# hassony2/homan

Measured on AMD Instinct MI355X. Metric: optimisation iters/sec (30-frame 256^2 clip), higher is better.
Workload: dtype f32

## Files before the change

### homan_amd/csrc/geometry.hip

```cpp
#include "hm_common.h"

__global__ __launch_bounds__(256) void k_rigid_fwd(const float* __restrict__ mesh, const float* __restrict__ rot6d,
                                                   const float* __restrict__ trans, const float* __restrict__ scale,
                                                   int abs_scale, int N, int V, float* __restrict__ rotmat,
                                                   float* __restrict__ verts, int clip_len)
{
    __shared__ float R[9];
    const int n = blockIdx.y;
    if (threadIdx.x == 0) {
        float r[9];
        rot6d_to_mat(rot6d + n * 6, r);
#pragma unroll
        for (int k = 0; k < 9; ++k) R[k] = r[k];
        if (blockIdx.x == 0 && rotmat)
#pragma unroll
            for (int k = 0; k < 9; ++k) rotmat[n * 9 + k] = r[k];
    }
    __syncthreads();
    const int v = blockIdx.x * blockDim.x + threadIdx.x;
    if (v >= V) return;
    float s = scale[n / clip_len];
    if (abs_scale) s = fabsf(s);
    const float* m = mesh + ((long)n * V + v) * 3;
    const float x = s * m[0], y = s * m[1], z = s * m[2];
// ... 140 lines not shown
        __syncthreads();
        if (threadIdx.x == 0) {
#pragma unroll
            for (int k = 0; k < 13; ++k) tot[k] = 0.f;
            for (unsigned c = 0; c < gridDim.y; ++c)
#pragma unroll
                for (int k = 0; k < 13; ++k) tot[k] += red13[c * 13 + k];
        }
    }
    }
    if (threadIdx.x == 0) {
        float dr6[6];
        rot6d_backward(rot6d + n * 6, tot, dr6);
#pragma unroll
        for (int k = 0; k < 6; ++k) g_rot6d[n * 6 + k] = dr6[k];
#pragma unroll
        for (int k = 0; k < 3; ++k) g_trans[n * 3 + k] = tot[9 + k];
        if (g_scale_part) g_scale_part[n] = (abs_scale && sraw < 0.f) ? -tot[12] : tot[12];
    }
    HM_STAMP_END(sil.parts ? 1 : 0);
}

struct SmoothIn { const float* verts; float w; };
template <int NV, int MAXT>
__global__ __launch_bounds__(MAXT) void k_rigid_bwd_x(const float* __restrict__ mesh, const float* __restrict__ rot6d,
                                                     const float* __restrict__ scale, int abs_scale, RigidTerms terms,
                                                     SilGather sil, SmoothIn sm, int N, int V, float* __restrict__ g_rot6d,
                                                     float* __restrict__ g_trans, float* __restrict__ g_scale_part,
                                                     float* __restrict__ partials, unsigned int* __restrict__ frame_cnt,
                                                     int clip_len, double magic)
{
    HM_LATENCY_KERNEL();
    HM_STAMP_START(1);
    __shared__ double red13d[16 * 13];
    __shared__ int s_flag;
    const int n = blockIdx.x;
    float R[9];
    rot6d_to_mat(rot6d + n * 6, R);
    const float sraw = scale[n / clip_len];
    const float s = abs_scale ? fabsf(sraw) : sraw;
    const int fl = n % clip_len;
    const long row = (long)V * 3;
    const long scnt = (long)(clip_len - 1) * row;
    const float inv_cnt = scnt > 0 ? 1.0f / (float)scnt : 0.f;
    int vv[NV];
    bool ok[NV];
    int a0[NV], a1[NV];
    float m[NV][3], cv[NV][3], tv[NV][5][3], nb[NV][2][3];
#pragma unroll
    for (int j = 0; j < NV; ++j) {
        vv[j] = ((int)blockIdx.y * NV + j) * (int)blockDim.x + (int)threadIdx.x;
        ok[j] = vv[j] < V;
        const int v = ok[j] ? vv[j] : 0;
        const long o = ((long)n * V + v) * 3;
        a0[j] = sil.parts ? sil.adj_off[v] : 0;
        a1[j] = sil.parts ? sil.adj_off[v + 1] : 0;
#pragma unroll
        for (int c = 0; c < 3; ++c) {
            m[j][c] = mesh[o + c];
            cv[j][c] = sil.parts ? sil.cam_verts[o + c] : 0.f;
        }
#pragma unroll
        for (int k = 0; k < 5; ++k)
#pragma unroll
            for (int c = 0; c < 3; ++c) tv[j][k][c] = terms.p[k] ? terms.p[k][o + c] : 0.f;
#pragma unroll
        for (int c = 0; c < 3; ++c) {
            nb[j][0][c] = (sm.verts && fl + 1 < clip_len) ? sm.verts[o + row + c] : 0.f;
            nb[j][1][c] = (sm.verts && fl >= 1) ? sm.verts[o - row + c] : 0.f;
        }
    }
    float sv[NV][3];
#pragma unroll
    for (int j = 0; j < NV; ++j)
#pragma unroll
        for (int c = 0; c < 3; ++c) sv[j][c] = sm.verts ? sm.verts[((long)n * V + (ok[j] ? vv[j] : 0)) * 3 + c] : 0.f;
    int item[NV][8];
#pragma unroll
    for (int j = 0; j < NV; ++j)
#pragma unroll
        for (int k = 0; k < 8; ++k) item[j][k] = (ok[j] && a0[j] + k < a1[j]) ? sil.adj_items[a0[j] + k] : -1;
    double su[NV], sw[NV];
    {
        const double2* pf = reinterpret_cast<const double2*>(sil.parts + (long)n * sil.F * 6);
        double2 g2[NV][8];
#pragma unroll
        for (int j = 0; j < NV; ++j)
#pragma unroll
            for (int k = 0; k < 8; ++k) g2[j][k] = item[j][k] >= 0 ? pf[item[j][k]] : make_double2(0.0, 0.0);
#pragma unroll
        for (int j = 0; j < NV; ++j) {
            su[j] = 0.0; sw[j] = 0.0;
#pragma unroll
            for (int k = 0; k < 8; ++k) { su[j] += g2[j][k].x; sw[j] += g2[j][k].y; }
            for (int a = a0[j] + 8; ok[j] && a < a1[j]; ++a) {
                const double2 g = pf[sil.adj_items[a]];
                su[j] += g.x; sw[j] += g.y;
            }
        }
    }
    double accd[13];
#pragma unroll
    for (int k = 0; k < 13; ++k) accd[k] = 0.0;
#pragma unroll
    for (int j = 0; j < NV; ++j) {
        if (!ok[j]) continue;
        float gf[3] = {0.f, 0.f, 0.f}, gt[3];
        if (sm.verts) {
#pragma unroll
            for (int c = 0; c < 3; ++c) {
                float g = 0.f;
                if (fl + 1 < clip_len) { const float d = nb[j][0][c] - sv[j][c]; g -= d; }
                if (fl >= 1) g += sv[j][c] - nb[j][1][c];
                gf[c] += sm.w * (2.0f * g * inv_cnt);
            }
        }
#pragma unroll
        for (int k = 0; k < 5; ++k)
            if (terms.p[k]) {
                gf[0] += terms.w[k] * tv[j][k][0]; gf[1] += terms.w[k] * tv[j][k][1]; gf[2] += terms.w[k] * tv[j][k][2];
            }
        if (sil.parts) {
            const float gu = (float)su[j], gv = (float)sw[j];
            const float* k = sil.K + n * 9;
            const float x = cv[j][0], y = cv[j][1], z = cv[j][2];
            const float zz = z + 1e-9f;
            const float du0 = gu * (2.0f / sil.orig_size), dv0 = -gv * (2.0f / sil.orig_size);
            const float dxn = k[0] * du0 + k[3] * dv0;
            const float dyn = k[1] * du0 + k[4] * dv0;
            gf[0] += dxn / zz;
            gf[1] += dyn / zz;
            gf[2] += -(dxn * x + dyn * y) / (zz * zz);
        }
        gt[0] = gf[0] + 0.f; gt[1] = gf[1] + 0.f; gt[2] = gf[2] + 0.f;
        const float dm[3] = {R[0] * gf[0] + R[1] * gf[1] + R[2] * gf[2], R[3] * gf[0] + R[4] * gf[1] + R[5] * gf[2],
                             R[6] * gf[0] + R[7] * gf[1] + R[8] * gf[2]};
#pragma unroll
        for (int i = 0; i < 3; ++i)
#pragma unroll
            for (int q = 0; q < 3; ++q) accd[3 * i + q] += hm_quant((s * m[j][i]) * gt[q], magic);
#pragma unroll
        for (int q = 0; q < 3; ++q) accd[9 + q] += hm_quant(gt[q], magic);
        accd[12] += hm_quant(m[j][0] * dm[0] + m[j][1] * dm[1] + m[j][2] * dm[2], magic);
    }
    hm_block_sum_n_f64<13>(accd, red13d);
    if (gridDim.y > 1) {
        double* rec = reinterpret_cast<double*>(partials + ((long)n * gridDim.y + blockIdx.y) * 32);
        if (threadIdx.x == 0) {
#pragma unroll
            for (int k = 0; k < 13; ++k) __hip_atomic_store(rec + k, accd[k], __ATOMIC_RELAXED, __HIP_MEMORY_SCOPE_AGENT);
        }
        if (!hm_last_block(frame_cnt + n, gridDim.y, &s_flag)) return;
        if (threadIdx.x < 13 * gridDim.y)
            red13d[threadIdx.x] = __hip_atomic_load(reinterpret_cast<const double*>(partials + ((long)n * gridDim.y + threadIdx.x / 13) * 32) + threadIdx.x % 13,
                                                    __ATOMIC_RELAXED, __HIP_MEMORY_SCOPE_AGENT);
        __syncthreads();
        if (threadIdx.x == 0) {
#pragma unroll
            for (int k = 0; k < 13; ++k) accd[k] = 0.0;
            for (unsigned c = 0; c < gridDim.y; ++c)
#pragma unroll
                for (int k = 0; k < 13; ++k) accd[k] += red13d[c * 13 + k];
        }
    }
    if (threadIdx.x == 0) {
        float tot[13], dr6[6];
#pragma unroll
        for (int k = 0; k < 13; ++k) tot[k] = (float)accd[k];
        rot6d_backward(rot6d + n * 6, tot, dr6);
#pragma unroll
        for (int k = 0; k < 6; ++k) g_rot6d[n * 6 + k] = dr6[k];
#pragma unroll
        for (int k = 0; k < 3; ++k) g_trans[n * 3 + k] = tot[9 + k];
        if (g_scale_part) g_scale_part[n] = (abs_scale && sraw < 0.f) ? -tot[12] : tot[12];
    }
    HM_STAMP_END(1);
}

__global__ void k_scale_by(const float* __restrict__ in, const float* __restrict__ s, long n, float* __restrict__ out)
{
    const long i = (long)blockIdx.x * blockDim.x + threadIdx.x;
    if (i < n) out[i] = s[0] * in[i];
}
__global__ void k_sum_small(const float* __restrict__ parts, int n, float w0, const float* __restrict__ extra, float w1,
                            float* __restrict__ out)
{
    __shared__ float red[16];
    const int c = blockIdx.x;
    float a = 0.f;
    for (int i = threadIdx.x; i < n; i += blockDim.x) a += parts[(long)c * n + i];
    a = hm_block_sum(a, red);
    if (threadIdx.x == 0) out[c] = w0 * a + (extra ? w1 * extra[c] : 0.f);
}

extern "C" {
int hm_sum_small_clips(const float* parts, int n, float w0, const float* extra, float w1, float* out, int nclips,
                       hipStream_t stream)
{
    HM_CHECK_ARG(parts && out && n > 0 && nclips > 0);
    hipLaunchKernelGGL(k_sum_small, dim3(nclips), dim3(64), 0, stream, parts, n, w0, extra, w1, out);
    return hm_launch_status();
}
int hm_rigid_fwd_clips(const float* mesh, const float* rot6d, const float* trans, const float* scale, int abs_scale, int N,
                       int V, float* rotmat, float* verts, int clip_len, hipStream_t stream)
{
    HM_CHECK_ARG(mesh && rot6d && trans && scale && verts && N > 0 && V > 0 && HM_CLIP_LEN_OK(N, clip_len));
    hipLaunchKernelGGL(k_rigid_fwd, dim3(hm_cdiv(V, 256), N), dim3(256), 0, stream, mesh, rot6d, trans, scale,
                       abs_scale, N, V, rotmat, verts, clip_len ? clip_len : N);
    return hm_launch_status();
}
int hm_rigid_fwd(const float* mesh, const float* rot6d, const float* trans, const float* scale, int abs_scale, int N,
                 int V, float* rotmat, float* verts, hipStream_t stream)
{
    return hm_rigid_fwd_clips(mesh, rot6d, trans, scale, abs_scale, N, V, rotmat, verts, 0, stream);
}
#define RIGID_MAX_CHUNKS 16
size_t hm_rigid_workspace_bytes(int N) { return (((size_t)N * 4 + 255) & ~(size_t)255) + (size_t)N * RIGID_MAX_CHUNKS * 32 * 4; }
static int rigid_bwd_launch(const float* mesh, const float* rot6d, const float* scale, int abs_scale,
                            const float* const* g_terms, const float* weights, int n_terms, SilGather sil,
                            const float* g_rigid, const float* g_frame, int frame_stride, float frame_scale, int N, int V,
                            float* g_mesh, float* g_rot6d, float* g_trans, float* g_scale_part, void* workspace,
                            int clip_len, int exact, int sum_log2q, SmoothIn smooth, hipStream_t stream)
{
    HM_CHECK_ARG(sum_log2q <= 0 && sum_log2q >= -60);
    HM_CHECK_ARG(mesh && rot6d && scale && g_rot6d && g_trans && N > 0 && V > 0 && HM_CLIP_LEN_OK(N, clip_len));
    HM_CHECK_ARG(n_terms >= 0 && n_terms <= 5 && (n_terms == 0 || (g_terms && weights)));
    HM_CHECK_ARG(!g_frame || frame_stride >= 3);
    HM_CHECK_ARG(HM_ALIGNED(workspace, 8));
    RigidTerms t;
    for (int k = 0; k < 5; ++k) { t.p[k] = k < n_terms ? g_terms[k] : nullptr; t.w[k] = k < n_terms ? weights[k] : 0.f; }
    const int threads = exact ? 256 : (V > 512 ? 1024 : 256);
    const int chunks = workspace ? min(RIGID_MAX_CHUNKS, hm_cdiv(V, exact ? threads : 4 * threads)) : 1;
    unsigned int* cnt = (unsigned int*)workspace;
    float* partials = workspace ? (float*)((char*)workspace + (((size_t)N * 4 + 255) & ~(size_t)255)) : nullptr;
    const bool small = V <= RIGID_MAX_CHUNKS * 256;
    const int nv = small ? 1 : 2;
    const int thr = small ? 256 : 768;
    if (exact && !g_rigid && !g_frame && !g_mesh && (workspace ? V <= RIGID_MAX_CHUNKS * thr * nv : V <= thr * nv)) {
        const int ch = hm_cdiv(V, thr * nv);
// ... 54 lines not shown
                     const float* weights, int n_terms, const double* sil_parts, const int* adj_off, const int* adj_items,
                     const float* cam_verts, const float* K, float orig_size, int F, int N, int V, float* g_rot6d,
                     float* g_trans, float* g_scale_part, void* workspace, int sum_log2q, hipStream_t stream)
{
    return hm_rigid_bwd_sil_clips(mesh, rot6d, scale, abs_scale, g_terms, weights, n_terms, sil_parts, adj_off, adj_items,
                                  cam_verts, K, orig_size, F, N, V, g_rot6d, g_trans, g_scale_part, workspace, 0, sum_log2q,
                                  nullptr, 0.f, stream);
}
int hm_scale_by(const float* in, const float* s, long n, float* out, hipStream_t stream)
{
    HM_CHECK_ARG(in && s && out && n > 0);
    hipLaunchKernelGGL(k_scale_by, dim3(hm_cdiv(n, 256)), dim3(256), 0, stream, in, s, n, out);
    return hm_launch_status();
}
#ifdef HM_CHAIN_STAMPS
int hm_debug_chain_geometry(unsigned long long* out, int reset)
{
    unsigned long long z[8] = {~0ull, 0, ~0ull, 0, ~0ull, 0, ~0ull, 0};
    (void)hipDeviceSynchronize();
    if (out) (void)hipMemcpyFromSymbol(out, HIP_SYMBOL(g_chain_ts), sizeof(z));
    if (reset) (void)hipMemcpyToSymbol(HIP_SYMBOL(g_chain_ts), z, sizeof(z));
    return HM_OK;
}
#endif
}
```

### homan_amd/csrc/hm_common.h

```cpp
#pragma once
#include <hip/hip_runtime.h>
#include <stdint.h>
#include "homan_amd.h"

#define HM_WAVE 64

#ifndef HM_PRIO
#define HM_PRIO 3
#endif
#define HM_LATENCY_KERNEL() __builtin_amdgcn_s_setprio(HM_PRIO)
#ifdef HM_CHAIN_STAMPS
static __device__ unsigned long long g_chain_ts[8];
#define HM_STAMP_START(k) do { if (threadIdx.x == 0) atomicMin(&g_chain_ts[2 * (k)], (unsigned long long)wall_clock64()); } while (0)
#define HM_STAMP_END(k) do { if (threadIdx.x == 0) atomicMax(&g_chain_ts[2 * (k) + 1], (unsigned long long)wall_clock64()); } while (0)
#else
#define HM_STAMP_START(k)
#define HM_STAMP_END(k)
#endif
#ifndef HM_HAND_PRIO
#define HM_HAND_PRIO HM_PRIO
#endif
#define HM_HAND_KERNEL() __builtin_amdgcn_s_setprio(HM_HAND_PRIO)
#ifdef HM_CHAIN_PRIO
#define HM_CHAIN_KERNEL() __builtin_amdgcn_s_setprio(HM_CHAIN_PRIO)
#else
#define HM_CHAIN_KERNEL()
#endif

#define HM_CHECK_ARG(cond) \
    do {                   \
        if (!(cond)) return HM_ERR_BAD_ARG; \
    } while (0)
#define HM_ALIGNED(p, bytes) ((((uintptr_t)(p)) & (uintptr_t)((bytes) - 1)) == 0)

#define HM_CLIP_LEN_OK(N, clip_len) ((clip_len) == 0 || ((clip_len) > 0 && (N) % (clip_len) == 0))
#define HM_RED_WS_FLOATS 576

static inline int hm_launch_status()
{
    hipError_t e = hipGetLastError();
// ... 335 lines not shown
```

### homan_amd/csrc/mano.hip

```cpp
#include "hm_common.h"
#include <string.h>

#define MANO_V 778
#define MANO_J 16
#define MANO_NF 145
#define MANO_CHUNK 256
#define MANO_NCHUNK 4
#define MANO_PART 352
#define MANO_NCH64 13
#define MANO_STATE_SH 832
#define MANO_STATE_DW (MANO_STATE_SH + 3 * MANO_V + 2)

struct ManoModelDev {
    const float* v_template;
    const float* M;
    const float* J_template;
    const float* J_shapedirs;
    const float* weights;
    const float* comps;
    const float* hand_mean;
    const int* parents;
};

__device__ __forceinline__ void rodrigues(const float* r, float* R)
// ... 145 lines not shown
    const int lane = threadIdx.x & 63, wv = threadIdx.x >> 6;
    const int v = min(v0 + lane, MANO_V - 1);
    float a0 = 0.f, a1 = 0.f, a2 = 0.f;
    const int k0 = wv * MANO_ROWS_PER_WAVE, k1 = min(MANO_NF, k0 + MANO_ROWS_PER_WAVE);
    const float* base = m.M + 3 * v;
#pragma unroll 4
    for (int k = k0; k < k1; ++k) {
        const float f = sh.feat[k];
        const float* row = base + (long)k * (3 * MANO_V);
        a0 += f * row[0];
        a1 += f * row[1];
        a2 += f * row[2];
    }
    s_part[wv][lane][0] = a0; s_part[wv][lane][1] = a1; s_part[wv][lane][2] = a2;
    __syncthreads();
    if (wv == 0) {
#pragma unroll
        for (int c = 0; c < 3; ++c)
            s_vp[lane][c] = m.v_template[3 * v + c] + ((s_part[0][lane][c] + s_part[1][lane][c]) + (s_part[2][lane][c] + s_part[3][lane][c]));
    }
    __syncthreads();
}

__device__ __forceinline__ void mano_skin_transform(const ManoModelDev& m, const ManoShared& sh, int v, float* T)
{
#pragma unroll
    for (int k = 0; k < 12; ++k) T[k] = 0.f;
    const float4* wrow = reinterpret_cast<const float4*>(m.weights + v * MANO_J);
#pragma unroll
    for (int q = 0; q < 4; ++q) {
        const float4 w4 = wrow[q];
        const float ws[4] = {w4.x, w4.y, w4.z, w4.w};
#pragma unroll
        for (int u = 0; u < 4; ++u) {
            const int j = 4 * q + u;
#pragma unroll
            for (int k = 0; k < 12; ++k) T[k] += ws[u] * sh.A[j][k];
        }
    }
}

#define MANO_FPW 4
__global__ __launch_bounds__(256) void k_mano_fwd(ManoModelDev m, const float* __restrict__ pca, int pca_stride,
                                                   const float* __restrict__ rot, const float* __restrict__ betas,
                                                   const float* __restrict__ trans, int B, float* __restrict__ verts,
                                                   float* __restrict__ joints, const float* __restrict__ rigid_rot6d,
// ... 60 lines not shown
    const float* vp = s_vp[wv][lane];
    float* o = verts + ((long)b * MANO_V + v) * 3;
    float p[3];
#pragma unroll
    for (int i = 0; i < 3; ++i) { p[i] = T[4 * i] * vp[0] + T[4 * i + 1] * vp[1] + T[4 * i + 2] * vp[2] + T[4 * i + 3] + tr[i]; o[i] = p[i]; }
    if (verts_world) {
        const float s = rigid_scale[b / clip_len];
        const float x = s * p[0], y = s * p[1], z = s * p[2];
        const float* t = rigid_trans + b * 3;
        const float* R = s_R[wv];
        float* ow = verts_world + ((long)b * MANO_V + v) * 3;
        ow[0] = x * R[0] + y * R[3] + z * R[6] + t[0];
        ow[1] = x * R[1] + y * R[4] + z * R[7] + t[1];
        ow[2] = x * R[2] + y * R[5] + z * R[8] + t[2];
    }
}

static_assert(sizeof(ManoShared) / 4 <= MANO_STATE_SH, "MANO_STATE_SH too small");

struct ManoBwd2Shared {
    float tot[MANO_PART];
    float dRw[MANO_J][9], dtw[MANO_J][3], dJ[MANO_J][3], dRl[MANO_J][9], dpose[48];
    float cR[MANO_J][9], ct[MANO_J][3], cJ[MANO_J][3];
};
__device__ __forceinline__ void mano_bwd2_body(const ManoModelDev& m, const ManoShared& sh, ManoBwd2Shared& w,
                                               const float* __restrict__ partials, int nchunk, int lb, int b, int pca_dim,
                                               const float* __restrict__ g_pca_extra, float w_extra,
                                               float* __restrict__ g_pca, float* __restrict__ g_rot,
                                               float* __restrict__ g_betas, float* __restrict__ g_trans)
{
    const int t = threadIdx.x, nt = blockDim.x;
    for (int k = t; k < MANO_PART; k += nt) {
        float v[MANO_NCH64];
#pragma unroll
        for (int c = 0; c < MANO_NCH64; ++c)
            v[c] = c < nchunk ? hm_partial_load(partials + ((long)lb * nchunk + c) * MANO_PART + k) : 0.f;
        float a = 0.f;
#pragma unroll
        for (int c = 0; c < MANO_NCH64; ++c) a += v[c];
        w.tot[k] = a;
    }
    int depth = 0, par = -1, maxd = 0;
    if (t < MANO_J) { par = sh.parents[t]; depth = sh.depth[t]; }
#pragma unroll
    for (int j = 0; j < MANO_J; ++j) maxd = max(maxd, sh.depth[j]);
    __syncthreads();
    if (t < MANO_J) {
        const int j = t;
        const float* dA = &w.tot[j * 12];
#pragma unroll
        for (int i = 0; i < 3; ++i) {
#pragma unroll
            for (int k = 0; k < 3; ++k) w.dRw[j][3 * i + k] = dA[4 * i + k] - dA[4 * i + 3] * sh.J[j][k];
            w.dtw[j][i] = dA[4 * i + 3];
        }
#pragma unroll
        for (int k = 0; k < 3; ++k)
            w.dJ[j][k] = -(sh.Rw[j][k] * dA[3] + sh.Rw[j][3 + k] * dA[7] + sh.Rw[j][6 + k] * dA[11]);
    }
    __syncthreads();
    for (int level = maxd; level >= 1; --level) {
        if (t < MANO_J && depth == level) {
            const int j = t, p = par;
            const float rel[3] = {sh.J[j][0] - sh.J[p][0], sh.J[j][1] - sh.J[p][1], sh.J[j][2] - sh.J[p][2]};
// ... 16 lines not shown
#pragma unroll
                for (int k = 0; k < 3; ++k)
                    w.dRl[j][3 * i + k] = sh.Rw[p][i] * w.dRw[j][k] + sh.Rw[p][3 + i] * w.dRw[j][3 + k] + sh.Rw[p][6 + i] * w.dRw[j][6 + k];
        }
        __syncthreads();
        if (t < MANO_J && depth == level - 1) {
            for (int j = 0; j < MANO_J; ++j)
                if (sh.parents[j] == t) {
#pragma unroll
                    for (int k = 0; k < 9; ++k) w.dRw[t][k] += w.cR[j][k];
#pragma unroll
                    for (int k = 0; k < 3; ++k) { w.dtw[t][k] += w.ct[j][k]; w.dJ[t][k] += w.cJ[j][k]; }
                }
        }
        __syncthreads();
    }
    if (t < MANO_J && par < 0) {
#pragma unroll
        for (int k = 0; k < 9; ++k) w.dRl[t][k] = w.dRw[t][k];
#pragma unroll
        for (int c = 0; c < 3; ++c) w.dJ[t][c] += w.dtw[t][c];
    }
    __syncthreads();
    if (t < MANO_J) {
        float dR[9];
#pragma unroll
        for (int k = 0; k < 9; ++k) dR[k] = w.dRl[t][k] + (t >= 1 ? w.tot[192 + 9 * (t - 1) + k] : 0.f);
        float dr[3];
        rodrigues_backward(&sh.pose[3 * t], dR, dr);
#pragma unroll
        for (int c = 0; c < 3; ++c) w.dpose[3 * t + c] = dr[c];
    }
    __syncthreads();
    if (t < 3) {
        g_rot[b * 3 + t] = w.dpose[t];
        g_trans[b * 3 + t] = w.tot[337 + t];
    }
    for (int i = t; i < pca_dim; i += nt) {
        float a = 0.f;
        if (i < 16) {
            float cv[45];
#pragma unroll
            for (int k = 0; k < 45; ++k) cv[k] = m.comps[i * 45 + k];
#pragma unroll
            for (int k = 0; k < 45; ++k) a += cv[k] * w.dpose[3 + k];
        }
        if (g_pca_extra) a += w_extra * g_pca_extra[(long)b * pca_dim + i];
        g_pca[(long)b * pca_dim + i] = a;
    }
    if (t < 10) {
        float a = w.tot[192 + 135 + t];
        float jv[MANO_J * 3];
#pragma unroll
        for (int q = 0; q < MANO_J * 3; ++q) jv[q] = m.J_shapedirs[q * 10 + t];
#pragma unroll
        for (int q = 0; q < MANO_J * 3; ++q) a += jv[q] * w.dJ[q / 3][q % 3];
        g_betas[b * 10 + t] = a;
    }
}

#ifdef MANO_PHASES
static __device__ unsigned long long g_mano_ph[16];
#define MPH_MARK(k) do { if (threadIdx.x == 0) { const unsigned long long t_ = wall_clock64(); atomicAdd(&g_mano_ph[k], t_ - mph_t); mph_t = t_; } } while (0)
#else
#define MPH_MARK(k)
#endif
struct ManoRigid {
    const float* mesh;
    const float* rot6d;
    const float* scale;
    int clip_len;
    RigidTerms terms;
    const float* g_rigid;
    const float* g_frame;
    int frame_stride;
    float frame_scale;
    float* g_rot6d; float* g_trans;
};
template <bool RIGID>
__global__ __launch_bounds__(256) void k_mano_bwd(ManoModelDev m, const float* __restrict__ pca, int pca_stride,
                                                   const float* __restrict__ rot, const float* __restrict__ betas,
                                                   const float* __restrict__ gout, int B, const float* __restrict__ state,
                                                   float* __restrict__ partials, unsigned int* __restrict__ frame_cnt,
                                                   int pca_dim, const float* __restrict__ g_pca_extra, float w_extra,
                                                   float* __restrict__ g_pca, float* __restrict__ g_rot,
                                                   float* __restrict__ g_betas, float* __restrict__ g_trans, int row0,
                                                   int row_stride, ManoRigid mr)
{
    HM_HAND_KERNEL();
    __shared__ ManoShared sh;
    __shared__ float s_part[4][MANO_VCH][3];
    __shared__ float s_vp[MANO_VCH][3];
    __shared__ float s_g[MANO_VCH][3];
    __shared__ float s_dvp[MANO_VCH * 3];
    __shared__ float s_w[MANO_VCH][MANO_J + 1];
    __shared__ float red[16];
    __shared__ ManoBwd2Shared w2;
    __shared__ int s_flag;
    const int lb = blockIdx.y, b = lb * row_stride + row0, t = threadIdx.x;
    const int v0 = blockIdx.x * MANO_VCH;
    const int nv = min(MANO_VCH, MANO_V - v0);
#ifdef MANO_PHASES
    unsigned long long mph_t = wall_clock64();
    if (t == 0) atomicAdd(&g_mano_ph[15], 1ull);
#endif
    if (state) {
        const float* st = state + (long)b * MANO_STATE_DW;
        for (int i = t; i < (int)(sizeof(ManoShared) / 4); i += blockDim.x) reinterpret_cast<float*>(&sh)[i] = st[i];
        if (t < 3 * nv) (&s_vp[0][0])[t] = st[MANO_STATE_SH + 3 * v0 + t];
        __syncthreads();
    } else {
        mano_prepare(m, pca, pca_stride, rot, betas, b, sh, threadIdx.x);
        mano_posed_chunk(m, sh, v0, s_part, s_vp);
    }
    MPH_MARK(0);
    float g[3] = {0.f, 0.f, 0.f};
    float racc[12];
#pragma unroll
    for (int k = 0; k < 12; ++k) racc[k] = 0.f;
    if (t < nv) {
        const int v = v0 + t;
        if (RIGID) {
            const long o = ((long)b * MANO_V + v) * 3;
            float R[9];
            rot6d_to_mat(mr.rot6d + (long)b * 6, R);
            const float s = mr.scale[b / mr.clip_len];
            const float mv[3] = {mr.mesh[o], mr.mesh[o + 1], mr.mesh[o + 2]};
            float gf[3] = {0.f, 0.f, 0.f}, gt[3];
#pragma unroll
            for (int k = 0; k < 5; ++k)
                if (mr.terms.p[k]) {
                    gf[0] += mr.terms.w[k] * mr.terms.p[k][o]; gf[1] += mr.terms.w[k] * mr.terms.p[k][o + 1];
                    gf[2] += mr.terms.w[k] * mr.terms.p[k][o + 2];
                }
#pragma unroll
            for (int c = 0; c < 3; ++c)
                gt[c] = gf[c] + (mr.g_frame ? mr.frame_scale * mr.g_frame[(long)b * mr.frame_stride + c] : 0.f);
            if (mr.g_rigid) { gt[0] += mr.g_rigid[o]; gt[1] += mr.g_rigid[o + 1]; gt[2] += mr.g_rigid[o + 2]; }
#pragma unroll
            for (int i = 0; i < 3; ++i)
#pragma unroll
                for (int j = 0; j < 3; ++j) racc[3 * i + j] = (s * mv[i]) * gt[j];
#pragma unroll
            for (int j = 0; j < 3; ++j) racc[9 + j] = gt[j];
            g[0] = s * (R[0] * gf[0] + R[1] * gf[1] + R[2] * gf[2]);
            g[1] = s * (R[3] * gf[0] + R[4] * gf[1] + R[5] * gf[2]);
            g[2] = s * (R[6] * gf[0] + R[7] * gf[1] + R[8] * gf[2]);
        } else {
            const float* gp = gout + ((long)b * MANO_V + v) * 3;
            g[0] = gp[0]; g[1] = gp[1]; g[2] = gp[2];
        }
    }
    float* out = partials + ((long)lb * gridDim.x + blockIdx.x) * MANO_PART;
    if (RIGID) {
        float* red12 = &s_part[0][0][0];
        hm_block_sum_n<12>(racc, red12);
        if (t < 12) hm_partial_store(out + 340 + t, racc[t]);
        __syncthreads();
    }
    if (t < nv) {
        const int v = v0 + t;
        float T[12];
        mano_skin_transform(m, sh, v, T);
#pragma unroll
        for (int c = 0; c < 3; ++c) {
            s_g[t][c] = g[c];
            s_dvp[3 * t + c] = T[c] * g[0] + T[4 + c] * g[1] + T[8 + c] * g[2];
        }
        for (int j = 0; j < MANO_J; ++j) s_w[t][j] = m.weights[v * MANO_J + j];
    }
    MPH_MARK(1);
    const float tg0 = hm_block_sum(g[0], red), tg1 = hm_block_sum(g[1], red), tg2 = hm_block_sum(g[2], red);
    if (t == 0) { hm_partial_store(out + 337, tg0); hm_partial_store(out + 338, tg1); hm_partial_store(out + 339, tg2); }
    __syncthreads();
    MPH_MARK(2);
    if (t < 192) {
        const int j = t / 12, r = (t % 12) / 4, c = t % 4;
        float acc = 0.f;
        for (int i = 0; i < nv; ++i) acc += s_w[i][j] * s_g[i][r] * (c < 3 ? s_vp[i][c] : 1.0f);
        hm_partial_store(out + t, acc);
    }
    __syncthreads();
    MPH_MARK(3);
    const int wv = t >> 6, lane = t & 63;
    const int ne = 3 * nv;
    float d0 = 0.f, d1 = 0.f, d2 = 0.f;
    if (lane < ne) d0 = s_dvp[lane];
    if (lane + 64 < ne) d1 = s_dvp[lane + 64];
    if (lane + 128 < ne) d2 = s_dvp[lane + 128];
    constexpr int ROWS = (MANO_NF + 3) / 4;
    float r0[ROWS], r1[ROWS], r2[ROWS];
#pragma unroll
    for (int q = 0; q < ROWS; ++q) {
        const int k = wv + 4 * q;
        const float* row = m.M + (long)min(k, MANO_NF - 1) * (3 * MANO_V) + 3 * v0;
        r0[q] = lane < ne ? row[lane] : 0.f;
        r1[q] = lane + 64 < ne ? row[lane + 64] : 0.f;
        r2[q] = lane + 128 < ne ? row[lane + 128] : 0.f;
    }
#pragma unroll
    for (int q = 0; q < ROWS; ++q) {
        const int k = wv + 4 * q;
        float acc = r0[q] * d0;
        acc += r1[q] * d1;
        acc += r2[q] * d2;
        acc = hm_wave_sum(acc);
        if (lane == 0 && k < MANO_NF) hm_partial_store(out + 192 + k, acc);
    }
    asm volatile("s_waitcnt vmcnt(0)" ::: "memory");
    __syncthreads();
    MPH_MARK(4);
    if (t == 0) {
        const unsigned int ticket = atomicAdd(frame_cnt + lb, 1u);
        const int last = ticket == gridDim.x - 1u;
        if (last) atomicExch(frame_cnt + lb, 0u);
        s_flag = last;
    }
    __syncthreads();
    MPH_MARK(5);
    if (s_flag) {
        mano_bwd2_body(m, sh, w2, partials, gridDim.x, lb, b, pca_dim, g_pca_extra, w_extra, g_pca, g_rot, g_betas, g_trans);
        if (RIGID) {
            __syncthreads();
            if (t == 0) {
                float dr6[6];
                rot6d_backward(mr.rot6d + (long)b * 6, &w2.tot[340], dr6);
#pragma unroll
                for (int k = 0; k < 6; ++k) mr.g_rot6d[(long)b * 6 + k] = dr6[k];
#pragma unroll
                for (int k = 0; k < 3; ++k) mr.g_trans[(long)b * 3 + k] = w2.tot[349 + k];
            }
        }
#ifdef MANO_PHASES
        __syncthreads();
        MPH_MARK(6);
        if (t == 0) atomicAdd(&g_mano_ph[14], 1ull);
#endif
    }
}

extern "C" {
int hm_mano_fwd_rows(const void* const* model, const float* pca, int pca_dim, const float* rot, const float* betas,
                     const float* trans, int B, float* verts, float* joints, const float* rigid_rot6d,
                     const float* rigid_trans, const float* rigid_scale, float* verts_world, float* state, int clip_len,
                     int row0, int row_stride, hipStream_t stream)
{
    HM_CHECK_ARG(model && pca && rot && betas && verts && B > 0 && pca_dim >= 16 && row_stride >= 1 && row0 >= 0 && row0 < row_stride);
    HM_CHECK_ARG(clip_len >= 0 && (clip_len == 0 || (B * row_stride) % clip_len == 0));
    HM_CHECK_ARG(!verts_world || (rigid_rot6d && rigid_trans && rigid_scale));
    HM_CHECK_ARG(HM_ALIGNED(model[4], 16));
    ManoModelDev m = {(const float*)model[0], (const float*)model[1], (const float*)model[2], (const float*)model[3],
                      (const float*)model[4], (const float*)model[5], (const float*)model[6], (const int*)model[7]};
    hipLaunchKernelGGL(k_mano_fwd, dim3(MANO_NCH64, (B + MANO_FPW - 1) / MANO_FPW), dim3(256), 0, stream, m, pca, pca_dim, rot, betas, trans, B, verts,
                       joints, rigid_rot6d, rigid_trans, rigid_scale, verts_world, state, clip_len ? clip_len : B * row_stride,
                       row0, row_stride);
    return hm_launch_status();
}
int hm_mano_fwd_clips(const void* const* model, const float* pca, int pca_dim, const float* rot, const float* betas,
                      const float* trans, int B, float* verts, float* joints, const float* rigid_rot6d,
                      const float* rigid_trans, const float* rigid_scale, float* verts_world, float* state, int clip_len,
                      hipStream_t stream)
// ... 10 lines not shown
int hm_mano_fwd(const void* const* model, const float* pca, int pca_dim, const float* rot, const float* betas,
                const float* trans, int B, float* verts, float* joints, const float* rigid_rot6d, const float* rigid_trans,
                const float* rigid_scale, float* verts_world, float* state, hipStream_t stream)
{
    return hm_mano_fwd_clips(model, pca, pca_dim, rot, betas, trans, B, verts, joints, rigid_rot6d, rigid_trans,
                             rigid_scale, verts_world, state, 0, stream);
}
size_t hm_mano_workspace_bytes(int B) { return 512 + (size_t)B * 4 + (size_t)B * MANO_NCH64 * MANO_PART * sizeof(float); }
size_t hm_mano_state_bytes(int B) { return (size_t)B * MANO_STATE_DW * sizeof(float); }
static int mano_bwd_launch(const void* const* model, const float* pca, int pca_dim, const float* rot, const float* betas, int B,
                           const float* g_verts, const float* g_pca_extra, float w_extra, float* g_pca, float* g_rot,
                           float* g_betas, float* g_trans, const float* state, void* workspace, int row0, int row_stride,
                           const ManoRigid& mr, hipStream_t stream)
{
    HM_CHECK_ARG(model && pca && rot && betas && (g_verts || mr.mesh) && g_pca && g_rot && g_betas && g_trans && workspace);
    HM_CHECK_ARG(HM_ALIGNED(workspace, 4));
    HM_CHECK_ARG(B > 0 && pca_dim >= 16 && row_stride >= 1 && row0 >= 0 && row0 < row_stride);
    HM_CHECK_ARG(HM_ALIGNED(model[4], 16));
    ManoModelDev m = {(const float*)model[0], (const float*)model[1], (const float*)model[2], (const float*)model[3],
                      (const float*)model[4], (const float*)model[5], (const float*)model[6], (const int*)model[7]};
    unsigned int* cnt = (unsigned int*)workspace;
    float* partials = (float*)((char*)workspace + 256 + (((size_t)B * 4 + 255) & ~(size_t)255));
    if (mr.mesh)
        hipLaunchKernelGGL(k_mano_bwd<true>, dim3(MANO_NCH64, B), dim3(256), 0, stream, m, pca, pca_dim, rot, betas,
                           g_verts, B, state, partials, cnt, pca_dim, g_pca_extra, w_extra, g_pca, g_rot, g_betas, g_trans, row0,
                           row_stride, mr);
    else
        hipLaunchKernelGGL(k_mano_bwd<false>, dim3(MANO_NCH64, B), dim3(256), 0, stream, m, pca, pca_dim, rot, betas,
                           g_verts, B, state, partials, cnt, pca_dim, g_pca_extra, w_extra, g_pca, g_rot, g_betas, g_trans, row0,
                           row_stride, mr);
    return hm_launch_status();
}
int hm_mano_bwd_rows(const void* const* model, const float* pca, int pca_dim, const float* rot, const float* betas, int B,
                     const float* g_verts, const float* g_pca_extra, float w_extra, float* g_pca, float* g_rot, float* g_betas,
                     float* g_trans, const float* state, void* workspace, int row0, int row_stride, hipStream_t stream)
{
    ManoRigid none;
    memset(&none, 0, sizeof(none));
    return mano_bwd_launch(model, pca, pca_dim, rot, betas, B, g_verts, g_pca_extra, w_extra, g_pca, g_rot, g_betas, g_trans,
                           state, workspace, row0, row_stride, none, stream);
}
int hm_mano_bwd_rigid_clips(const void* const* model, const float* pca, int pca_dim, const float* rot, const float* betas, int B,
                            const float* g_pca_extra, float w_extra, float* g_pca, float* g_rot, float* g_betas,
                            float* g_trans, const float* state, void* workspace, const float* mesh, const float* rigid_rot6d,
                            const float* rigid_scale, const float* const* g_terms, const float* weights, int n_terms,
                            const float* g_rigid, const float* g_frame, int frame_stride, float frame_scale,
                            float* g_rigid_rot6d, float* g_rigid_trans, int clip_len, hipStream_t stream)
{
    HM_CHECK_ARG(mesh && rigid_rot6d && rigid_scale && g_rigid_rot6d && g_rigid_trans && HM_CLIP_LEN_OK(B, clip_len));
    HM_CHECK_ARG(n_terms >= 0 && n_terms <= 5 && (n_terms == 0 || (g_terms && weights)));
    HM_CHECK_ARG(!g_frame || frame_stride >= 3);
// ... 2 lines not shown
    mr.mesh = mesh; mr.rot6d = rigid_rot6d; mr.scale = rigid_scale; mr.clip_len = clip_len ? clip_len : B;
    for (int k = 0; k < 5; ++k) { mr.terms.p[k] = k < n_terms ? g_terms[k] : nullptr; mr.terms.w[k] = k < n_terms ? weights[k] : 0.f; }
    mr.g_rigid = g_rigid; mr.g_frame = g_frame; mr.frame_stride = frame_stride; mr.frame_scale = frame_scale;
    mr.g_rot6d = g_rigid_rot6d; mr.g_trans = g_rigid_trans;
    return mano_bwd_launch(model, pca, pca_dim, rot, betas, B, nullptr, g_pca_extra, w_extra, g_pca, g_rot, g_betas, g_trans,
                           state, workspace, 0, 1, mr, stream);
}
int hm_mano_bwd(const void* const* model, const float* pca, int pca_dim, const float* rot, const float* betas, int B,
                const float* g_verts, const float* g_pca_extra, float w_extra, float* g_pca, float* g_rot, float* g_betas,
                float* g_trans, const float* state, void* workspace, hipStream_t stream)
{
    return hm_mano_bwd_rows(model, pca, pca_dim, rot, betas, B, g_verts, g_pca_extra, w_extra, g_pca, g_rot, g_betas, g_trans,
                            state, workspace, 0, 1, stream);
}
#ifdef MANO_PHASES
int hm_debug_mano_phases(unsigned long long* out)
{
    unsigned long long z[16] = {0};
    (void)hipDeviceSynchronize();
    (void)hipMemcpyFromSymbol(out, HIP_SYMBOL(g_mano_ph), sizeof(z));
    (void)hipMemcpyToSymbol(HIP_SYMBOL(g_mano_ph), z, sizeof(z));
    return HM_OK;
}
#endif
}
```

Before: 6748.

## Shorten reduction tails in rigid and MANO backward kernels

```diff
diff --git a/homan_amd/csrc/geometry.hip b/homan_amd/csrc/geometry.hip
--- a/homan_amd/csrc/geometry.hip
+++ b/homan_amd/csrc/geometry.hip
@@ -186,6 +186,17 @@
 }
 
 struct SmoothIn { const float* verts; float w; };
+#define RIGID_MAX_CHUNKS 16
+#ifdef HM_CHAIN_STAMPS
+static __device__ unsigned long long g_tail_ph[16];
+#define RPH_DECL() HM_PH_DECL()
+#define RPH(k) HM_PH(k)
+#define RPH_FLUSH() HM_PH_FLUSH(g_tail_ph)
+#else
+#define RPH_DECL()
+#define RPH(k)
+#define RPH_FLUSH()
+#endif
 template <int NV, int MAXT>
 __global__ __launch_bounds__(MAXT) void k_rigid_bwd_x(const float* __restrict__ mesh, const float* __restrict__ rot6d,
                                                      const float* __restrict__ scale, int abs_scale, RigidTerms terms,
@@ -196,11 +207,14 @@
 {
     HM_LATENCY_KERNEL();
     HM_STAMP_START(1);
+    RPH_DECL();
+    RPH(0);
     __shared__ double red13d[16 * 13];
-    __shared__ int s_flag;
     const int n = blockIdx.x;
-    float R[9];
-    rot6d_to_mat(rot6d + n * 6, R);
+    float r6[6], R[9];
+#pragma unroll
+    for (int k = 0; k < 6; ++k) r6[k] = rot6d[n * 6 + k];
+    rot6d_to_mat(r6, R);
     const float sraw = scale[n / clip_len];
     const float s = abs_scale ? fabsf(sraw) : sraw;
     const int fl = n % clip_len;
@@ -239,11 +253,13 @@
     for (int j = 0; j < NV; ++j)
 #pragma unroll
         for (int c = 0; c < 3; ++c) sv[j][c] = sm.verts ? sm.verts[((long)n * V + (ok[j] ? vv[j] : 0)) * 3 + c] : 0.f;
+    RPH(1);
     int item[NV][8];
 #pragma unroll
     for (int j = 0; j < NV; ++j)
 #pragma unroll
         for (int k = 0; k < 8; ++k) item[j][k] = (ok[j] && a0[j] + k < a1[j]) ? sil.adj_items[a0[j] + k] : -1;
+    RPH(2);
     double su[NV], sw[NV];
     {
         const double2* pf = reinterpret_cast<const double2*>(sil.parts + (long)n * sil.F * 6);
@@ -263,6 +279,7 @@
             }
         }
     }
+    RPH(3);
     double accd[13];
 #pragma unroll
     for (int k = 0; k < 13; ++k) accd[k] = 0.0;
@@ -308,36 +325,52 @@
         accd[12] += hm_quant(m[j][0] * dm[0] + m[j][1] * dm[1] + m[j][2] * dm[2], magic);
     }
     hm_block_sum_n_f64<13>(accd, red13d);
+    RPH(4);
+    if (threadIdx.x >= HM_WAVE) return;
     if (gridDim.y > 1) {
-        double* rec = reinterpret_cast<double*>(partials + ((long)n * gridDim.y + blockIdx.y) * 32);
+        double mine = 0.0;
+#pragma unroll
+        for (int k = 0; k < 13; ++k) mine = (int)threadIdx.x == k ? accd[k] : mine;
+        if (threadIdx.x < 13)
+            __hip_atomic_store(reinterpret_cast<double*>(partials + ((long)n * gridDim.y + blockIdx.y) * 32) + threadIdx.x, mine,
+                               __ATOMIC_RELAXED, __HIP_MEMORY_SCOPE_AGENT);
+        RPH(5);
+        unsigned int ticket = 0;
         if (threadIdx.x == 0) {
-#pragma unroll
-            for (int k = 0; k < 13; ++k) __hip_atomic_store(rec + k, accd[k], __ATOMIC_RELAXED, __HIP_MEMORY_SCOPE_AGENT);
-        }
-        if (!hm_last_block(frame_cnt + n, gridDim.y, &s_flag)) return;
-        if (threadIdx.x < 13 * gridDim.y)
-            red13d[threadIdx.x] = __hip_atomic_load(reinterpret_cast<const double*>(partials + ((long)n * gridDim.y + threadIdx.x / 13) * 32) + threadIdx.x % 13,
-                                                    __ATOMIC_RELAXED, __HIP_MEMORY_SCOPE_AGENT);
-        __syncthreads();
-        if (threadIdx.x == 0) {
-#pragma unroll
-            for (int k = 0; k < 13; ++k) accd[k] = 0.0;
-            for (unsigned c = 0; c < gridDim.y; ++c)
-#pragma unroll
-                for (int k = 0; k < 13; ++k) accd[k] += red13d[c * 13 + k];
-        }
+            asm volatile("s_waitcnt vmcnt(0)" ::: "memory");
+            ticket = atomicAdd(frame_cnt + n, 1u);
+            if (ticket == gridDim.y - 1u) atomicExch(frame_cnt + n, 0u);
+        }
+        ticket = (unsigned int)__builtin_amdgcn_readfirstlane((int)ticket);
+        asm volatile("" ::: "memory");
+        RPH(6);
+        if (ticket != gridDim.y - 1u) { RPH_FLUSH(); return; }
+        double part[RIGID_MAX_CHUNKS];
+        const double* recs = reinterpret_cast<const double*>(partials + (long)n * gridDim.y * 32) + (threadIdx.x < 13 ? threadIdx.x : 0);
+#pragma unroll
+        for (int c = 0; c < RIGID_MAX_CHUNKS; ++c)
+            part[c] = c < (int)gridDim.y ? __hip_atomic_load(recs + c * 16, __ATOMIC_RELAXED, __HIP_MEMORY_SCOPE_AGENT) : 0.0;
+        mine = 0.0;
+#pragma unroll
+        for (int c = 0; c < RIGID_MAX_CHUNKS; ++c) mine += part[c];
+        RPH(7);
+#pragma unroll
+        for (int k = 0; k < 13; ++k)
+            accd[k] = __hiloint2double(__builtin_amdgcn_readlane(__double2hiint(mine), k), __builtin_amdgcn_readlane(__double2loint(mine), k));
     }
     if (threadIdx.x == 0) {
         float tot[13], dr6[6];
 #pragma unroll
         for (int k = 0; k < 13; ++k) tot[k] = (float)accd[k];
-        rot6d_backward(rot6d + n * 6, tot, dr6);
+        rot6d_backward(r6, tot, dr6);
 #pragma unroll
         for (int k = 0; k < 6; ++k) g_rot6d[n * 6 + k] = dr6[k];
 #pragma unroll
         for (int k = 0; k < 3; ++k) g_trans[n * 3 + k] = tot[9 + k];
         if (g_scale_part) g_scale_part[n] = (abs_scale && sraw < 0.f) ? -tot[12] : tot[12];
     }
+    RPH(8);
+    RPH_FLUSH();
     HM_STAMP_END(1);
 }
 
@@ -378,7 +411,6 @@
 {
     return hm_rigid_fwd_clips(mesh, rot6d, trans, scale, abs_scale, N, V, rotmat, verts, 0, stream);
 }
-#define RIGID_MAX_CHUNKS 16
 size_t hm_rigid_workspace_bytes(int N) { return (((size_t)N * 4 + 255) & ~(size_t)255) + (size_t)N * RIGID_MAX_CHUNKS * 32 * 4; }
 static int rigid_bwd_launch(const float* mesh, const float* rot6d, const float* scale, int abs_scale,
                             const float* const* g_terms, const float* weights, int n_terms, SilGather sil,
@@ -479,5 +511,14 @@
     if (reset) (void)hipMemcpyToSymbol(HIP_SYMBOL(g_chain_ts), z, sizeof(z));
     return HM_OK;
 }
+int hm_debug_tail_geometry(unsigned long long* out, int reset)
+{
+    unsigned long long z[16] = {0};
+    z[15] = ~0ull;
+    (void)hipDeviceSynchronize();
+    if (out) (void)hipMemcpyFromSymbol(out, HIP_SYMBOL(g_tail_ph), sizeof(z));
+    if (reset) (void)hipMemcpyToSymbol(HIP_SYMBOL(g_tail_ph), z, sizeof(z));
+    return HM_OK;
+}
 #endif
 }
diff --git a/homan_amd/csrc/hm_common.h b/homan_amd/csrc/hm_common.h
--- a/homan_amd/csrc/hm_common.h
+++ b/homan_amd/csrc/hm_common.h
@@ -16,6 +16,12 @@
 #else
 #define HM_STAMP_START(k)
 #define HM_STAMP_END(k)
+#endif
+#if defined(HM_CHAIN_STAMPS) || defined(MANO_PHASES)
+#define HM_PH_DECL() unsigned long long ph_[15] = {}
+#define HM_PH(k) do { asm volatile("s_waitcnt vmcnt(0) lgkmcnt(0)" ::: "memory"); ph_[k] = wall_clock64(); } while (0)
+#define HM_PH_FLUSH(arr) do { if (threadIdx.x == 0) { atomicMin(&(arr)[15], ph_[0]); \
+        for (int k_ = 0; k_ < 15; ++k_) if (ph_[k_]) atomicMax(&(arr)[k_], ph_[k_]); } } while (0)
 #endif
 #ifndef HM_HAND_PRIO
 #define HM_HAND_PRIO HM_PRIO
diff --git a/homan_amd/csrc/mano.hip b/homan_amd/csrc/mano.hip
--- a/homan_amd/csrc/mano.hip
+++ b/homan_amd/csrc/mano.hip
@@ -191,6 +191,22 @@
     __syncthreads();
 }
 
+__device__ __forceinline__ void mano_skin_transform_w(const ManoShared& sh, const float4* wrow, float* T)
+{
+#pragma unroll
+    for (int k = 0; k < 12; ++k) T[k] = 0.f;
+#pragma unroll
+    for (int q = 0; q < 4; ++q) {
+        const float4 w4 = wrow[q];
+        const float ws[4] = {w4.x, w4.y, w4.z, w4.w};
+#pragma unroll
+        for (int u = 0; u < 4; ++u) {
+            const int j = 4 * q + u;
+#pragma unroll
+            for (int k = 0; k < 12; ++k) T[k] += ws[u] * sh.A[j][k];
+        }
+    }
+}
 __device__ __forceinline__ void mano_skin_transform(const ManoModelDev& m, const ManoShared& sh, int v, float* T)
 {
 #pragma unroll
@@ -297,24 +313,66 @@
     float tot[MANO_PART];
     float dRw[MANO_J][9], dtw[MANO_J][3], dJ[MANO_J][3], dRl[MANO_J][9], dpose[48];
     float cR[MANO_J][9], ct[MANO_J][3], cJ[MANO_J][3];
+    float comps[MANO_J * 45], jsd[MANO_J * 3 * 10];
 };
+struct ManoRigid;
+__device__ __forceinline__ void mano_rigid_finish(const ManoRigid& mr, const float* r6, const float* tot12, int b);
+#ifdef MANO_PHASES
+static __device__ unsigned long long g_mano_tail[16];
+#define TPH_DECL() HM_PH_DECL()
+#define TPH(k) HM_PH(k)
+#define TPH_FLUSH() HM_PH_FLUSH(g_mano_tail)
+#define TPH_ARG , unsigned long long (&ph_)[15]
+#define TPH_PASS , ph_
+#else
+#define TPH_DECL()
+#define TPH(k)
+#define TPH_FLUSH()
+#define TPH_ARG
+#define TPH_PASS
+#endif
+#define MANO_BWD_THREADS 256
+template <bool RIGID>
 __device__ __forceinline__ void mano_bwd2_body(const ManoModelDev& m, const ManoShared& sh, ManoBwd2Shared& w,
                                                const float* __restrict__ partials, int nchunk, int lb, int b, int pca_dim,
                                                const float* __restrict__ g_pca_extra, float w_extra,
                                                float* __restrict__ g_pca, float* __restrict__ g_rot,
-                                               float* __restrict__ g_betas, float* __restrict__ g_trans)
-{
-    const int t = threadIdx.x, nt = blockDim.x;
-    for (int k = t; k < MANO_PART; k += nt) {
-        float v[MANO_NCH64];
-#pragma unroll
-        for (int c = 0; c < MANO_NCH64; ++c)
-            v[c] = c < nchunk ? hm_partial_load(partials + ((long)lb * nchunk + c) * MANO_PART + k) : 0.f;
-        float a = 0.f;
-#pragma unroll
-        for (int c = 0; c < MANO_NCH64; ++c) a += v[c];
-        w.tot[k] = a;
-    }
+                                               float* __restrict__ g_betas, float* __restrict__ g_trans, const ManoRigid& mr,
+                                               const float* r6 TPH_ARG)
+{
+    const int t = threadIdx.x, nt = MANO_BWD_THREADS;
+    static_assert(MANO_PART <= 2 * MANO_BWD_THREADS, "two passes over the chunk records");
+    constexpr int NSTAGE = MANO_J * 45 + MANO_J * 3 * 10, SPT = (NSTAGE + MANO_BWD_THREADS - 1) / MANO_BWD_THREADS;
+    const float ex = (g_pca_extra && t < pca_dim) ? g_pca_extra[(long)b * pca_dim + t] : 0.f;
+    {
+        const bool two = t + nt < MANO_PART;
+        float v0[MANO_NCH64], v1[MANO_NCH64], stg[SPT];
+#pragma unroll
+        for (int c = 0; c < MANO_NCH64; ++c) {
+            const float* rec = partials + ((long)lb * nchunk + c) * MANO_PART + t;
+            v0[c] = c < nchunk ? hm_partial_load(rec) : 0.f;
+            v1[c] = (two && c < nchunk) ? hm_partial_load(rec + nt) : 0.f;
+        }
+#pragma unroll
+        for (int q = 0; q < SPT; ++q) {
+            const int i = t + q * nt;
+            stg[q] = i < MANO_J * 45 ? m.comps[i] : (i < NSTAGE ? m.J_shapedirs[i - MANO_J * 45] : 0.f);
+        }
+        float a0 = 0.f, a1 = 0.f;
+#pragma unroll
+        for (int c = 0; c < MANO_NCH64; ++c) a0 += v0[c];
+#pragma unroll
+        for (int c = 0; c < MANO_NCH64; ++c) a1 += v1[c];
+        w.tot[t] = a0;
+        if (two) w.tot[t + nt] = a1;
+#pragma unroll
+        for (int q = 0; q < SPT; ++q) {
+            const int i = t + q * nt;
+            if (i < MANO_J * 45) w.comps[i] = stg[q];
+            else if (i < NSTAGE) w.jsd[i - MANO_J * 45] = stg[q];
+        }
+    }
+    TPH(5);
     int depth = 0, par = -1, maxd = 0;
     if (t < MANO_J) { par = sh.parents[t]; depth = sh.depth[t]; }
 #pragma unroll
@@ -377,6 +435,7 @@
         for (int c = 0; c < 3; ++c) w.dJ[t][c] += w.dtw[t][c];
     }
     __syncthreads();
+    TPH(6);
     if (t < MANO_J) {
         float dR[9];
 #pragma unroll
@@ -385,8 +444,17 @@
         rodrigues_backward(&sh.pose[3 * t], dR, dr);
 #pragma unroll
         for (int c = 0; c < 3; ++c) w.dpose[3 * t + c] = dr[c];
-    }
-    __syncthreads();
+    } else if (t >= 2 * HM_WAVE && t < 2 * HM_WAVE + 10) {
+        const int l = t - 2 * HM_WAVE;
+        float a = w.tot[192 + 135 + l];
+#pragma unroll
+        for (int q = 0; q < MANO_J * 3; ++q) a += w.jsd[q * 10 + l] * w.dJ[q / 3][q % 3];
+        g_betas[b * 10 + l] = a;
+    } else if (RIGID && t == HM_WAVE) {
+        mano_rigid_finish(mr, r6, &w.tot[340], b);
+    }
+    __syncthreads();
+    TPH(7);
     if (t < 3) {
         g_rot[b * 3 + t] = w.dpose[t];
         g_trans[b * 3 + t] = w.tot[337 + t];
@@ -394,24 +462,13 @@
     for (int i = t; i < pca_dim; i += nt) {
         float a = 0.f;
         if (i < 16) {
-            float cv[45];
-#pragma unroll
-            for (int k = 0; k < 45; ++k) cv[k] = m.comps[i * 45 + k];
-#pragma unroll
-            for (int k = 0; k < 45; ++k) a += cv[k] * w.dpose[3 + k];
-        }
-        if (g_pca_extra) a += w_extra * g_pca_extra[(long)b * pca_dim + i];
+#pragma unroll
+            for (int k = 0; k < 45; ++k) a += w.comps[i * 45 + k] * w.dpose[3 + k];
+        }
+        if (g_pca_extra) a += w_extra * (i == t ? ex : g_pca_extra[(long)b * pca_dim + i]);
         g_pca[(long)b * pca_dim + i] = a;
     }
-    if (t < 10) {
-        float a = w.tot[192 + 135 + t];
-        float jv[MANO_J * 3];
-#pragma unroll
-        for (int q = 0; q < MANO_J * 3; ++q) jv[q] = m.J_shapedirs[q * 10 + t];
-#pragma unroll
-        for (int q = 0; q < MANO_J * 3; ++q) a += jv[q] * w.dJ[q / 3][q % 3];
-        g_betas[b * 10 + t] = a;
-    }
+    TPH(8);
 }
 
 #ifdef MANO_PHASES
@@ -432,8 +489,17 @@
     float frame_scale;
     float* g_rot6d; float* g_trans;
 };
+__device__ __forceinline__ void mano_rigid_finish(const ManoRigid& mr, const float* r6, const float* tot12, int b)
+{
+    float dr6[6];
+    rot6d_backward(r6, tot12, dr6);
+#pragma unroll
+    for (int k = 0; k < 6; ++k) mr.g_rot6d[(long)b * 6 + k] = dr6[k];
+#pragma unroll
+    for (int k = 0; k < 3; ++k) mr.g_trans[(long)b * 3 + k] = tot12[9 + k];
+}
 template <bool RIGID>
-__global__ __launch_bounds__(256) void k_mano_bwd(ManoModelDev m, const float* __restrict__ pca, int pca_stride,
+__global__ __launch_bounds__(MANO_BWD_THREADS) void k_mano_bwd(ManoModelDev m, const float* __restrict__ pca, int pca_stride,
                                                    const float* __restrict__ rot, const float* __restrict__ betas,
                                                    const float* __restrict__ gout, int B, const float* __restrict__ state,
                                                    float* __restrict__ partials, unsigned int* __restrict__ frame_cnt,
@@ -449,7 +515,6 @@
     __shared__ float s_g[MANO_VCH][3];
     __shared__ float s_dvp[MANO_VCH * 3];
     __shared__ float s_w[MANO_VCH][MANO_J + 1];
-    __shared__ float red[16];
     __shared__ ManoBwd2Shared w2;
     __shared__ int s_flag;
     const int lb = blockIdx.y, b = lb * row_stride + row0, t = threadIdx.x;
@@ -459,6 +524,31 @@
     unsigned long long mph_t = wall_clock64();
     if (t == 0) atomicAdd(&g_mano_ph[15], 1ull);
 #endif
+    TPH_DECL();
+    TPH(0);
+    const int vq = v0 + (t < nv ? t : 0);
+    const long o = ((long)b * MANO_V + vq) * 3;
+    float4 w4[4];
+#pragma unroll
+    for (int q = 0; q < 4; ++q) w4[q] = reinterpret_cast<const float4*>(m.weights + vq * MANO_J)[q];
+    float gin[3] = {0.f, 0.f, 0.f}, mv[3] = {0.f, 0.f, 0.f}, tv[5][3], gfr[3] = {0.f, 0.f, 0.f}, grg[3] = {0.f, 0.f, 0.f};
+    float r6[6] = {0.f, 0.f, 0.f, 0.f, 0.f, 0.f}, rs = 0.f;
+    if (RIGID) {
+#pragma unroll
+        for (int k = 0; k < 6; ++k) r6[k] = mr.rot6d[(long)b * 6 + k];
+        rs = mr.scale[b / mr.clip_len];
+#pragma unroll
+        for (int c = 0; c < 3; ++c) {
+            mv[c] = mr.mesh[o + c];
+#pragma unroll
+            for (int k = 0; k < 5; ++k) tv[k][c] = mr.terms.p[k] ? mr.terms.p[k][o + c] : 0.f;
+            if (mr.g_frame) gfr[c] = mr.g_frame[(long)b * mr.frame_stride + c];
+            if (mr.g_rigid) grg[c] = mr.g_rigid[o + c];
+        }
+    } else {
+#pragma unroll
+        for (int c = 0; c < 3; ++c) gin[c] = gout[o + c];
+    }
     if (state) {
         const float* st = state + (long)b * MANO_STATE_DW;
         for (int i = t; i < (int)(sizeof(ManoShared) / 4); i += blockDim.x) reinterpret_cast<float*>(&sh)[i] = st[i];
@@ -469,29 +559,27 @@
         mano_posed_chunk(m, sh, v0, s_part, s_vp);
     }
     MPH_MARK(0);
+    TPH(1);
     float g[3] = {0.f, 0.f, 0.f};
-    float racc[12];
-#pragma unroll
-    for (int k = 0; k < 12; ++k) racc[k] = 0.f;
+    float racc[15];
+#pragma unroll
+    for (int k = 0; k < 15; ++k) racc[k] = 0.f;
     if (t < nv) {
-        const int v = v0 + t;
         if (RIGID) {
-            const long o = ((long)b * MANO_V + v) * 3;
             float R[9];
-            rot6d_to_mat(mr.rot6d + (long)b * 6, R);
-            const float s = mr.scale[b / mr.clip_len];
-            const float mv[3] = {mr.mesh[o], mr.mesh[o + 1], mr.mesh[o + 2]};
+            rot6d_to_mat(r6, R);
+            const float s = rs;
             float gf[3] = {0.f, 0.f, 0.f}, gt[3];
 #pragma unroll
             for (int k = 0; k < 5; ++k)
                 if (mr.terms.p[k]) {
-                    gf[0] += mr.terms.w[k] * mr.terms.p[k][o]; gf[1] += mr.terms.w[k] * mr.terms.p[k][o + 1];
-                    gf[2] += mr.terms.w[k] * mr.terms.p[k][o + 2];
+                    gf[0] += mr.terms.w[k] * tv[k][0]; gf[1] += mr.terms.w[k] * tv[k][1];
+                    gf[2] += mr.terms.w[k] * tv[k][2];
                 }
 #pragma unroll
             for (int c = 0; c < 3; ++c)
-                gt[c] = gf[c] + (mr.g_frame ? mr.frame_scale * mr.g_frame[(long)b * mr.frame_stride + c] : 0.f);
-            if (mr.g_rigid) { gt[0] += mr.g_rigid[o]; gt[1] += mr.g_rigid[o + 1]; gt[2] += mr.g_rigid[o + 2]; }
+                gt[c] = gf[c] + (mr.g_frame ? mr.frame_scale * gfr[c] : 0.f);
+            if (mr.g_rigid) { gt[0] += grg[0]; gt[1] += grg[1]; gt[2] += grg[2]; }
 #pragma unroll
             for (int i = 0; i < 3; ++i)
 #pragma unroll
@@ -502,40 +590,47 @@
             g[1] = s * (R[3] * gf[0] + R[4] * gf[1] + R[5] * gf[2]);
             g[2] = s * (R[6] * gf[0] + R[7] * gf[1] + R[8] * gf[2]);
         } else {
-            const float* gp = gout + ((long)b * MANO_V + v) * 3;
-            g[0] = gp[0]; g[1] = gp[1]; g[2] = gp[2];
+            g[0] = gin[0]; g[1] = gin[1]; g[2] = gin[2];
         }
     }
     float* out = partials + ((long)lb * gridDim.x + blockIdx.x) * MANO_PART;
-    if (RIGID) {
-        float* red12 = &s_part[0][0][0];
-        hm_block_sum_n<12>(racc, red12);
-        if (t < 12) hm_partial_store(out + 340 + t, racc[t]);
-        __syncthreads();
-    }
+    {
+        float* red15 = &s_part[0][0][0];
+        float tg[3] = {g[0], g[1], g[2]};
+        if (RIGID) {
+#pragma unroll
+            for (int c = 0; c < 3; ++c) racc[12 + c] = g[c];
+            hm_block_sum_n<15>(racc, red15);
+            float mine = 0.f;
+#pragma unroll
+            for (int k = 0; k < 15; ++k) mine = t == k ? racc[k] : mine;
+            if (t < 15) hm_partial_store(out + (t < 12 ? 340 + t : 337 + (t - 12)), mine);
+        } else {
+            hm_block_sum_n<3>(tg, red15);
+            if (t == 0) { hm_partial_store(out + 337, tg[0]); hm_partial_store(out + 338, tg[1]); hm_partial_store(out + 339, tg[2]); }
+        }
+    }
+    MPH_MARK(1);
     if (t < nv) {
-        const int v = v0 + t;
         float T[12];
-        mano_skin_transform(m, sh, v, T);
+        mano_skin_transform_w(sh, w4, T);
 #pragma unroll
         for (int c = 0; c < 3; ++c) {
             s_g[t][c] = g[c];
             s_dvp[3 * t + c] = T[c] * g[0] + T[4 + c] * g[1] + T[8 + c] * g[2];
         }
-        for (int j = 0; j < MANO_J; ++j) s_w[t][j] = m.weights[v * MANO_J + j];
-    }
-    MPH_MARK(1);
-    const float tg0 = hm_block_sum(g[0], red), tg1 = hm_block_sum(g[1], red), tg2 = hm_block_sum(g[2], red);
-    if (t == 0) { hm_partial_store(out + 337, tg0); hm_partial_store(out + 338, tg1); hm_partial_store(out + 339, tg2); }
+#pragma unroll
+        for (int q = 0; q < 4; ++q) { s_w[t][4 * q] = w4[q].x; s_w[t][4 * q + 1] = w4[q].y; s_w[t][4 * q + 2] = w4[q].z; s_w[t][4 * q + 3] = w4[q].w; }
+    }
     __syncthreads();
     MPH_MARK(2);
+    TPH(2);
     if (t < 192) {
         const int j = t / 12, r = (t % 12) / 4, c = t % 4;
         float acc = 0.f;
         for (int i = 0; i < nv; ++i) acc += s_w[i][j] * s_g[i][r] * (c < 3 ? s_vp[i][c] : 1.0f);
         hm_partial_store(out + t, acc);
     }
-    __syncthreads();
     MPH_MARK(3);
     const int wv = t >> 6, lane = t & 63;
     const int ne = 3 * nv;
@@ -565,6 +660,7 @@
     asm volatile("s_waitcnt vmcnt(0)" ::: "memory");
     __syncthreads();
     MPH_MARK(4);
+    TPH(3);
     if (t == 0) {
         const unsigned int ticket = atomicAdd(frame_cnt + lb, 1u);
         const int last = ticket == gridDim.x - 1u;
@@ -573,25 +669,17 @@
     }
     __syncthreads();
     MPH_MARK(5);
+    TPH(4);
     if (s_flag) {
-        mano_bwd2_body(m, sh, w2, partials, gridDim.x, lb, b, pca_dim, g_pca_extra, w_extra, g_pca, g_rot, g_betas, g_trans);
-        if (RIGID) {
-            __syncthreads();
-            if (t == 0) {
-                float dr6[6];
-                rot6d_backward(mr.rot6d + (long)b * 6, &w2.tot[340], dr6);
-#pragma unroll
-                for (int k = 0; k < 6; ++k) mr.g_rot6d[(long)b * 6 + k] = dr6[k];
-#pragma unroll
-                for (int k = 0; k < 3; ++k) mr.g_trans[(long)b * 3 + k] = w2.tot[349 + k];
-            }
-        }
+        mano_bwd2_body<RIGID>(m, sh, w2, partials, gridDim.x, lb, b, pca_dim, g_pca_extra, w_extra, g_pca, g_rot, g_betas, g_trans,
+                              mr, r6 TPH_PASS);
 #ifdef MANO_PHASES
         __syncthreads();
         MPH_MARK(6);
         if (t == 0) atomicAdd(&g_mano_ph[14], 1ull);
 #endif
     }
+    TPH_FLUSH();
 }
 
 extern "C" {
@@ -648,11 +736,11 @@
     unsigned int* cnt = (unsigned int*)workspace;
     float* partials = (float*)((char*)workspace + 256 + (((size_t)B * 4 + 255) & ~(size_t)255));
     if (mr.mesh)
-        hipLaunchKernelGGL(k_mano_bwd<true>, dim3(MANO_NCH64, B), dim3(256), 0, stream, m, pca, pca_dim, rot, betas,
+        hipLaunchKernelGGL(k_mano_bwd<true>, dim3(MANO_NCH64, B), dim3(MANO_BWD_THREADS), 0, stream, m, pca, pca_dim, rot, betas,
                            g_verts, B, state, partials, cnt, pca_dim, g_pca_extra, w_extra, g_pca, g_rot, g_betas, g_trans, row0,
                            row_stride, mr);
     else
-        hipLaunchKernelGGL(k_mano_bwd<false>, dim3(MANO_NCH64, B), dim3(256), 0, stream, m, pca, pca_dim, rot, betas,
+        hipLaunchKernelGGL(k_mano_bwd<false>, dim3(MANO_NCH64, B), dim3(MANO_BWD_THREADS), 0, stream, m, pca, pca_dim, rot, betas,
                            g_verts, B, state, partials, cnt, pca_dim, g_pca_extra, w_extra, g_pca, g_rot, g_betas, g_trans, row0,
                            row_stride, mr);
     return hm_launch_status();
@@ -701,5 +789,14 @@
     (void)hipMemcpyToSymbol(HIP_SYMBOL(g_mano_ph), z, sizeof(z));
     return HM_OK;
 }
+int hm_debug_tail_mano(unsigned long long* out, int reset)
+{
+    unsigned long long z[16] = {0};
+    z[15] = ~0ull;
+    (void)hipDeviceSynchronize();
+    if (out) (void)hipMemcpyFromSymbol(out, HIP_SYMBOL(g_mano_tail), sizeof(z));
+    if (reset) (void)hipMemcpyToSymbol(HIP_SYMBOL(g_mano_tail), z, sizeof(z));
+    return HM_OK;
+}
 #endif
 }
```

After: 6824, median of 6. +1.1%, better.
